# stevenabreu7/SparseRNNs

Hardware: AMD Instinct MI355X
Metric: frames/sec at w8a16 S5 dim_scale=0.5 (NDNS shape), bit-exact vs CPU fxprun (higher is better)
Workload: dtype int32

## Files before the change

### include/s5fxp.h

```cpp
#ifndef S5FXP_H
#define S5FXP_H

#include <stddef.h>
#include <stdint.h>

#ifdef __cplusplus
extern "C" {
#endif

#define S5FXP_VERSION 108

enum {
    S5FXP_OK = 0,
    S5FXP_EBADARG = -1,
    S5FXP_ENEGSHIFT = -2,
    S5FXP_EUNSUPPORTED = -3,
    S5FXP_EHIP = -4,
    S5FXP_EWORKSPACE = -5
};

enum { S5FXP_FLOOR = 0, S5FXP_CEIL = 1, S5FXP_ROUND = 2 };

int s5fxp_version(void);
const char *s5fxp_strerror(int code);
// ... 94 lines not shown
typedef struct {
    int32_t *pre_s5;
    int32_t *u;
    int32_t *Bu_re, *Bu_im;
    int32_t *xs_re, *xs_im;
    int32_t *ys;
    int32_t *out2;
    int32_t *out2_sigmoid;
    int32_t *post_GLU;
    int32_t *residadd;
} s5fxp_layer_trace;

size_t s5fxp_model_blob_bytes(const s5fxp_model_desc *desc);

enum { S5FXP_MODEL_DEFAULT = 0, S5FXP_MODEL_FORCE_DENSE = 1, S5FXP_MODEL_FORCE_CSR = 2, S5FXP_MODEL_FORCE_GENERIC = 4,
       S5FXP_MODEL_NO_RESID_FOLD = 8 };
int s5fxp_model_create(const s5fxp_model_desc *desc, void *dev_blob, size_t blob_bytes, int flags, void *stream,
                       s5fxp_model **out);
void s5fxp_model_destroy(s5fxp_model *m);

size_t s5fxp_workspace_bytes(const s5fxp_model *m, int B, int L);

#define S5FXP_STATUS_WORDS 128
enum { S5FXP_PATH_GENERIC = 1, S5FXP_PATH_FUSED = 2, S5FXP_PATH_STEP = 3 };
enum {
    S5FXP_ST_NEGSHIFT = 1,
    S5FXP_ST_NEGEXP = 2,
    S5FXP_ST_WIDE_STATE = 4,
    S5FXP_ST_WIDE_INPUT = 8,
    S5FXP_ST_REDO = 16
};
// ... 50 lines not shown
```

### sparsernns_amd/_lib.py

```python
from __future__ import annotations

import ctypes as C
import os

import torch

_HERE = os.path.dirname(os.path.abspath(__file__))
LIB_PATH = os.environ.get("S5FXP_LIB") or os.path.join(_HERE, "libs5fxp.so")

I32P = C.POINTER(C.c_int32)
VOIDP = C.c_void_p

S5FXP_OK, S5FXP_EBADARG, S5FXP_ENEGSHIFT, S5FXP_EUNSUPPORTED, S5FXP_EHIP, S5FXP_EWORKSPACE = 0, -1, -2, -3, -4, -5
ST_NEGSHIFT, ST_NEGEXP, ST_WIDE_STATE, ST_WIDE_INPUT, ST_REDO = 1, 2, 4, 8, 16
FWD_DEFER_REDO, FWD_EXACT, FWD_NO_PAIR = 1, 2, 4
STATUS_WORDS = 128
PATH_GENERIC, PATH_FUSED, PATH_STEP = 1, 2, 3
STEP_MAX_ROWS = 32
STREAM_MAX_HOPS = 32
MODEL_DEFAULT, MODEL_FORCE_DENSE, MODEL_FORCE_CSR, MODEL_FORCE_GENERIC, MODEL_NO_RESID_FOLD = 0, 1, 2, 4, 8


class DenseDesc(C.Structure):
    _fields_ = [("K", C.c_int32), ("M", C.c_int32), ("weight", I32P), ("bias", I32P)] + [
        (n, C.c_int32) for n in ("w_bits", "w_exp", "b_bits", "b_exp", "inp_bits", "inp_exp", "out_bits", "out_exp")]


class SSMDesc(C.Structure):
    _fields_ = [("H", C.c_int32), ("P", C.c_int32)] + [
        (n, I32P) for n in ("A_re", "A_im", "B_re", "B_im", "C_re", "C_im", "D")] + [
        (n, C.c_int32) for n in (
            "A_re_bits", "A_re_exp", "A_im_bits", "A_im_exp", "B_re_bits", "B_re_exp", "B_im_bits", "B_im_exp",
            "C_re_bits", "C_re_exp", "C_im_bits", "C_im_exp", "D_bits", "D_exp",
            "u_bits", "u_exp", "Bu_re_bits", "Bu_re_exp", "Bu_im_bits", "Bu_im_exp",
            "x_re_bits", "x_re_exp", "x_im_bits", "x_im_exp", "y_bits", "y_exp")]
# ... 116 lines not shown
```

### sparsernns_amd/csrc/mfma_bn.hpp

```cpp
#pragma once
#include "mfma_proj.hpp"

namespace s5 {

struct StatusInit {
    int32_t path;
    int32_t rk[15];
    int32_t slots[15];
    int32_t stream[15];
};
__global__ __launch_bounds__(256) void k_clear2(int32_t *a, int na, int32_t *b, int nb, StatusInit si, int n_layers, GroupOff go)
{
    gshift(a, (int64_t)blockIdx.y * go.status);
    gshift(b, (int64_t)blockIdx.y * go.ws);
    for (int i = blockIdx.x * 256 + threadIdx.x; i < na + nb; i += gridDim.x * 256) {
        if (i < na) {
            int32_t v = 0;
            if (i == 2) v = si.path;
            else if (i >= 8 && (i & 7) == 5 && (i - 8) / 8 < n_layers) v = si.rk[(i - 8) / 8];
            else if (i >= 8 && (i & 7) == 6 && (i - 8) / 8 < n_layers) v = si.slots[(i - 8) / 8];
            else if (i >= 8 && (i & 7) == 7 && (i - 8) / 8 < n_layers) v = si.stream[(i - 8) / 8];
            a[i] = v;
        } else b[i - na] = 0;
    }
// ... 470 lines not shown
__device__ __forceinline__ uint32_t pk_mul_sat(uint32_t a, uint32_t m)
{
    uint32_t r;
    asm("v_pk_mad_i16 %0, %1, %2, 0 clamp" : "=v"(r) : "v"(a), "v"(m));
    return r;
}
__device__ __forceinline__ uint32_t sum_u16_pair(const SumU16 &p, uint32_t z, uint32_t s)
{
    const uint32_t a = pk_mul_sat(pk_mul_sat(z, p.mz), p.mz2), b = pk_mul_sat(pk_mul_sat(s, p.ms), p.ms2);
    const uint32_t m = pk_max(a, pk_sub_sat(0u, b));
    uint32_t r;
    asm("v_pk_add_u16 %0, %1, %2" : "=v"(r) : "v"(m), "v"(b));
    return r;
}

enum { ROW_GENERIC = 0, ROW_PACKED = 1, ROW_SHIFTED = 2 };
struct Bn16Row {
    uint32_t m[4], iv[4];
    int32_t arm;
    uint32_t mulx, mulc, crp;
    int32_t shx1, l1, r1, rs2, cl, cr;
    int32_t xb, b1, b2, cbits;
};

__host__ __device__ __forceinline__ int bn16_row_arm(int xb, int mb, int ib, int b1, int b2, int cbits, int shx1, int l1, int r1, int cl, int cr)
{
    const bool w16 = (xb == 16 || (shx1 == 0 && xb < 16)) && mb <= 16 && ib <= 16 && b1 == 16 && b2 == 16 && cbits == 16 &&
                     shx1 <= 14 && l1 == 0 && cl <= 14 && cr <= 15;
    return !w16 ? ROW_GENERIC : r1 == 0 ? ROW_PACKED : ROW_SHIFTED;
}
// ... 61 lines not shown
    const int16_t *x;
    MfmaW w;
    int32_t *bq;
    int16_t *u;
    int32_t *tr_bu_re, *tr_bu_im, *tr_pre_s5, *tr_u;
    int64_t N;
    int32_t L, TB, H, P;
    int32_t rs_re, rs_im, bre_bits, bim_bits, sh_re, sh_im;
    int32_t t_lo, t_len;
    int32_t k_re;
    int32_t no_u;
    int32_t live_slots;
    const float *ext;
    int32_t ext_reps;
    int32_t *status, *status_exps;
};

}
```

### sparsernns_amd/csrc/mfma_fused.hpp

```cpp
#pragma once
#include "proj_p.hpp"

namespace s5 {

using v2i16 = __attribute__((ext_vector_type(2))) short;

struct CGateArgs {
    const int16_t *u;
    BnArgs bn;
    const int16_t *skip;
    const int32_t *xs;
    MfmaW w_re, w_im;
    MfmaW w_o2;
    const int32_t *D;
    const int32_t *bias_eff;
    int16_t *z;
    int32_t *tr_ys, *tr_out2, *tr_sig, *tr_z;
    int64_t N;
    int32_t L, TB, H;
    int32_t rs_re, rs_im, rs_d, y_bits, y_exp;
    int32_t xmax;
    int32_t conv, inp_bits, inp_exp, rs_o2, out_bits, out_exp;
    int32_t sig_x, sig_y;
    int32_t lut[8];
// ... 41 lines not shown
        w[0] = b0 ? r01 : w[0]; w[1] = b0 ? w[1] : r01;
        w[2] = b0 ? r23 : w[2]; w[3] = b0 ? w[3] : r23;
    }
    {
        const int32_t r02 = quad_xchg<0x4E>(b1 ? w[0] : w[2]), r13 = quad_xchg<0x4E>(b1 ? w[1] : w[3]);
        w[0] = b1 ? r02 : w[0]; w[2] = b1 ? w[2] : r02;
        w[1] = b1 ? r13 : w[1]; w[3] = b1 ? w[3] : r13;
    }
}


constexpr int SIGTAB_WORDS = 2 * 7 * 64;
constexpr int SIGDIR_MAX_BITS = 12, SIGDIR_BYTES = 2 << SIGDIR_MAX_BITS;
__host__ __device__ __forceinline__ int sigdir_lds_bytes(int bits) { return ((2 << bits) + 15) & ~15; }

template <int KS, int NT, bool TRACE, bool S16 = false, bool DIRECT = false, int FTP = 64, bool WIDE = false, bool PAIR = false, bool PK16 = false,
          bool GBN = false, bool UREC = false>
#ifndef S5_CGATE_HID
#define S5_CGATE_HID 0
#endif
#ifndef S5_CGATE_COAL
#define S5_CGATE_COAL 1
#endif
#ifndef S5_CGATE_LB
#define S5_CGATE_LB 4
#endif
__global__ __launch_bounds__(FTP * 2 * NT, NT == 3 && KS == 1 && !WIDE ? S5_CGATE_LB : 3) void k_cgate_p(const CGateArgs a_k, GroupOff go)
{
    constexpr bool FOLD = false;
#include "mfma_fused_body.inc"
}
struct CGateFoldArgs : CGateArgs {};
template <int KS, int NT, bool TRACE, bool S16, bool DIRECT, int FTP, bool WIDE, bool PAIR, bool PK16, bool GBN, bool UREC>
__global__ __launch_bounds__(FTP * 2 * NT, NT == 3 && KS == 1 && !WIDE ? S5_CGATE_LB : 3) void k_cgate_p(const CGateFoldArgs a_k, GroupOff go)
{
    constexpr bool FOLD = true;
#include "mfma_fused_body.inc"
}

}
```

### sparsernns_amd/csrc/mfma_fused_body.inc

```
    CGateArgs a = a_k;
    {
        const int64_t g = blockIdx.y;
        gshift(a.u, g * go.ws); gshift(a.skip, g * go.ws); gshift(a.xs, g * go.ws); gshift(a.z, g * go.ws);
        gshift(a.skip_e.dyn, g * go.ws); gshift(a.dynw, g * go.ws); gshift(a.run_if, g * go.ws); gshift(a.status, g * go.status);
        if constexpr (GBN || UREC) { gshift(a.bn.dyn, g * go.ws); gshift(a.bn.xe.dyn, g * go.ws); }
    }
    static_assert(!GBN || (PK16 && !TRACE && !WIDE), "the BatchNorm rides on the packed-epilogue kernel only");
    static_assert(!UREC || (S5_CGATE_COAL && PK16 && !TRACE && !WIDE && !GBN && !(S5_CGATE_HID && S16 && PAIR && KS * NT < 24)),
                  "u is rebuilt in the row tiles' staging: COAL only");
    constexpr int P = 32 * KS, H = shape_channels(NT), HP = 32 * NT, FT = FTP, NW = (FT / 32) * NT, NTHR = 64 * NW;
    constexpr bool RAGGED = H != HP;
    constexpr int KPS = 2 * P + 16, KPX = HP + 16;
    constexpr int NU = 1, SUBSTEP = 0;
    constexpr int ITEMS = (FT / 4) * P, ROUNDS = (ITEMS + NTHR - 1) / NTHR;
    constexpr bool HID = S5_CGATE_HID && S16 && PAIR && PK16 && !WIDE && !TRACE && KS * NT < 24;
    extern __shared__ __attribute__((aligned(16))) int8_t smem[];
    int32_t *csr = reinterpret_cast<int32_t *>(smem), *csi = csr + HP, *Dl = csi + HP, *cs2 = Dl + HP, *be = cs2 + HP, *lutp = be + HP;
    int32_t *sigt = lutp + 8;
    const int16_t *sigd = reinterpret_cast<const int16_t *>(sigt);
    constexpr int NPL = WIDE ? 4 : 2;
    int8_t *Sbase = reinterpret_cast<int8_t *>(sigt) + (DIRECT ? sigdir_lds_bytes(a.sigdir_bits) : 4 * SIGTAB_WORDS);
    int8_t *Sl = Sbase, *Sh = Sbase + (NPL - 1) * FT * KPS, *Xh = Sbase + NPL * FT * KPS, *Xl = Xh + FT * KPX;
    float *red = reinterpret_cast<float *>(Xl + FT * KPX);
    int32_t *bntab = reinterpret_cast<int32_t *>(red + 48);
// ... 35 lines not shown
    } else {
        for (int i = threadIdx.x; i < (14 << a.sig_x); i += NTHR) sigt[i] = a.sigtab[i];
    }
    Bn16 bn{};
    if constexpr (GBN) bn = bn16_setup(a.bn, *a.bn.dyn, bntab, H);
    std::conditional_t<UREC, Bn16Row, int> brow{};
    if constexpr (UREC) brow = bn16_row_setup(a.bn, *a.bn.dyn, 8 * (int)(threadIdx.x % VPF));
    const int dsh = a.out_exp - a.sig_x, dbias = 1 << (a.sigdir_bits - 1);
    const int skip_e = a.skip_e.get();
    const float kz = ldexpf(1.f, skip_e - a.res_exp);
    const v4i *usum_lds = reinterpret_cast<const v4i *>(red + 8);
    if constexpr (FOLD) {
        if (threadIdx.x == 0) {
            const SumU16 us = sum_u16_setup_exps(a.res_exp, skip_e);
            *reinterpret_cast<v4i *>(red + 8) = v4i{(int)us.mz, (int)us.mz2, (int)us.ms, (int)us.ms2};
        }
    }
    const int sx = a.sig_x, S = 1 << sx;
    const int cv_l = a.conv && a.inp_exp > a.y_exp ? a.inp_exp - a.y_exp : 0, cv_r = a.conv && a.y_exp > a.inp_exp ? a.y_exp - a.inp_exp : 0;
    const int cv_b1 = a.conv && a.inp_exp != a.y_exp ? a.y_bits : 32, cv_b2 = a.conv && a.y_bits > a.inp_bits ? a.inp_bits : 32;
    const int cv_b = cv_b1 < cv_b2 ? cv_b1 : cv_b2;
    const int lq_l = a.l_exp > a.y_exp ? a.l_exp - a.y_exp : 0, lq_r = a.y_exp > a.l_exp ? a.y_exp - a.l_exp : 0;
    uint32_t xrange = 0;
    v2i16 pmax = {0, 0}, pmin = {0, 0};
    float mx[3] = {0.f, 0.f, 0.f};
    const int ch0 = 32 * ct + 4 * h;
    v2i uq[NU][4], sq[NU][4];
    v4i urow[COAL && !UREC ? NVC : 1], srow[COAL ? NVC : 1];
    auto load_tile = [&](v4i(&dst)[COAL ? NVC : 1], const int16_t *src, const TileWalk<FT> &tw) {
        const int64_t b = tw.b;
        const int t = tw.t(sr), nv = tw.nvalid(sr);
        const char *base = reinterpret_cast<const char *>(src + (b * a.L + t) * H);
// ... 97 lines not shown
            }
        }
    };
    auto tiles_in_urec = [&](auto arm_c) {
        constexpr int ARM = decltype(arm_c)::value;
#pragma unroll
        for (int i = 0; i < NVC; ++i) {
            const int v = threadIdx.x + NTHR * i, f = v / VPF, og = v % VPF;
            if (!NVC_FULL && v >= FT * VPF) break;
            int8_t *cu = Ut + f * TROW + 16 * og, *cs_ = St + f * TROW + 16 * og;
            if (zb_prev) {
                v2i z0 = *reinterpret_cast<const v2i *>(cu), z1 = *reinterpret_cast<const v2i *>(cu + 8);
                if constexpr (FOLD) fold_z(z0, z1, cs_);
                if (f < nvalid_prev) *reinterpret_cast<v4i *>(zb_prev + 2u * (unsigned)(f * H + 8 * og)) = v4i{z0[0], z0[1], z1[0], z1[1]};
            }
            const v4i uv = bn16_row8<ARM>(brow, srow[i]);
            *reinterpret_cast<v2i *>(cu) = v2i{uv[0], uv[1]};
            *reinterpret_cast<v2i *>(cu + 8) = v2i{uv[2], uv[3]};
            *reinterpret_cast<v2i *>(cs_) = v2i{srow[i][0], srow[i][1]};
            *reinterpret_cast<v2i *>(cs_ + 8) = v2i{srow[i][2], srow[i][3]};
        }
    };

    prologue_loads_done();
    for (int64_t tile = blockIdx.x; tile < tiles; tile += gridDim.x, walk.advance()) {
        const int64_t b0 = walk.b;
        const int t0 = walk.t(sr), nvalid = walk.nvalid(sr);
        const TileWalk<FT> walk_next = walk.next();
        const int64_t n0 = b0 * a.L + t0;
        char *zb = reinterpret_cast<char *>(a.z + n0 * H);
// ... 312 lines not shown
```

### sparsernns_amd/csrc/proj_p.hpp

```cpp
#pragma once
#ifdef S5_PHASE_PROF
__device__ long long g_phase_prof[2048 * 8];
#define PHASE_DECL unsigned prof_last, prof_a0 = 0, prof_a1 = 0, prof_a2 = 0, prof_a3 = 0, prof_a4 = 0, prof_a5 = 0, prof_a6 = 0, prof_a7 = 0; \
    { unsigned long long t_; asm volatile("s_memtime %0\n\ts_waitcnt lgkmcnt(0)" : "=s"(t_)); prof_last = __builtin_amdgcn_readfirstlane((unsigned)t_); }
#define PHASE_MARK(i, reg) do { unsigned long long t_; asm volatile("v_cmp_eq_u32 vcc, %1, %1\n\ts_nop 0\n\ts_memtime %0\n\ts_waitcnt lgkmcnt(0)" : "=s"(t_) : "v"(reg) : "memory", "vcc"); \
    const unsigned tl_ = __builtin_amdgcn_readfirstlane((unsigned)t_); prof_a##i = __builtin_amdgcn_readfirstlane(prof_a##i + (tl_ - prof_last)); prof_last = tl_; } while (0)
#define PHASE_DUMP do { if (threadIdx.x == 0 && blockIdx.x < 2048) { long long *o_ = g_phase_prof + blockIdx.x * 8; o_[0] = prof_a0; o_[1] = prof_a1; o_[2] = prof_a2; o_[3] = prof_a3; \
    o_[4] = prof_a4; o_[5] = prof_a5; o_[6] = prof_a6; o_[7] = prof_a7; } } while (0)
#else
#define PHASE_DECL
#define PHASE_MARK(i, reg)
#define PHASE_DUMP
#endif
#define PHASE_DECL_F
#define PHASE_MARK_F(i, reg)
#define PHASE_DUMP_F
#include "mfma_bn.hpp"

namespace s5 {

__host__ __device__ constexpr int shape_channels(int NT) { return (NT == 2 || NT == 5) ? 32 * NT - 16 : 32 * NT; }

template <int HC, int HP, int KP>
__device__ __forceinline__ void zero_plane_tail(int8_t *base, int rows)
// ... 108 lines not shown
    if (wsub == 0 && h == 0) {
        const int col = 32 * wct + r;
        int n = 0;
        for (int k = 0; k < H; ++k) {
            const int8_t wv = a.w.wt[(size_t)col * a.w.Kp + k];
            if (wv != 0 && n < ELLW) ell[col * ELLW + n++] = (uint16_t)(k | ((unsigned)(uint8_t)wv << 8));
        }
        for (int j = n; j < ELLW; ++j) ell[col * ELLW + j] = 0;
        atomicMax(ellmax + wct, n);
    }
#endif
    const LayerDyn d = a.ext ? bn_finalize_mm_body(a.bn, a.ext, H, const_cast<LayerDyn *>(a.bn.dyn), a.status, a.status_exps, a.bn.xe.get(), a.ext_reps,
                                                   blockIdx.x == 0)
                             : *a.bn.dyn;
    const Bn16 bn = bn16_setup(a.bn, d, tab, H);
    __syncthreads();

    prologue_loads_done();
    for (int it = 0; tile < tiles; tile += gridDim.x, ++it, walk.advance()) {
        const int64_t b0 = walk.b;
        const int t0 = walk.t(sr), nvalid = walk.nvalid(sr);
        const int64_t n0 = b0 * a.L + t0;
        char *ub = reinterpret_cast<char *>(a.u + n0 * H);
        int8_t *xh = Xh + (it & 1) * PLANE, *xl = Xl + (it & 1) * PLANE;
#pragma unroll
        for (int i = 0; i < NV; ++i) {
            const int v = threadIdx.x + NTHR * i, f = v / VPF, og = v % VPF;
            const int64_t n = n0 + f;
            int32_t xin[8], t[8], u[8];
            unpack8_i16(raw[i], xin);
            bn16_x4(bn, reinterpret_cast<const int32_t(&)[4]>(xin[0]), 8 * og, reinterpret_cast<int32_t(&)[4]>(t[0]),
                    reinterpret_cast<int32_t(&)[4]>(u[0]));
            bn16_x4(bn, reinterpret_cast<const int32_t(&)[4]>(xin[4]), 8 * og + 4, reinterpret_cast<int32_t(&)[4]>(t[4]),
                    reinterpret_cast<int32_t(&)[4]>(u[4]));
            if (f < nvalid && (TRACE || !a.no_u)) {
                const v2i p0 = pack4_i16(u[0], u[1], u[2], u[3]), p1 = pack4_i16(u[4], u[5], u[6], u[7]);
                *reinterpret_cast<v4i *>(ub + 2u * (unsigned)(f * H + 8 * og)) = v4i{p0[0], p0[1], p1[0], p1[1]};
                if (TRACE) {
#pragma unroll
                    for (int e = 0; e < 8; ++e) {
                        if (a.tr_pre_s5) a.tr_pre_s5[n * H + 8 * og + e] = t[e];
                        if (a.tr_u) a.tr_u[n * H + 8 * og + e] = u[e];
                    }
                }
// ... 856 lines not shown
```

### sparsernns_amd/csrc/s5fxp_fast.hpp

```cpp
#pragma once

namespace s5 {
struct StepParams;
}

struct MfmaWDev {
    MfmaW w{};
    const int32_t *bias_eff = nullptr;
};

struct FastLayer {
    MfmaWDev bproj, cre, cim, out2;
    MfmaWDev bproj_pair;
    const int32_t *Dpad = nullptr;
    const int32_t *sigtab = nullptr;
    const int16_t *sigdir = nullptr;
    int sigdir_bits = 0;
    bool bias16 = false;
    bool compact_ok = false;
    int n_live = 0;
    int c_slots = 0;
    MfmaWDev c_bproj, c_bproj_pair, c_cre, c_cim;
    ScanBounds c_bounds;
    const int32_t *c_a_re = nullptr, *c_a_im = nullptr;
// ... 279 lines not shown

struct LayerPlan {
    bool compact;
    Rung rung;
    int P;
    int ks;
    int live_slots;
    int stream_slots;
    int32_t bound;
    int32_t xmax;
    bool direct;
    bool pk16;
    bool gate_bn;
    bool gate_urec;
    bool resid_fold;
    GateForm gate;
    const MfmaW *w_bproj, *w_cre, *w_cim;
    const int32_t *a_re, *a_im;
};

LayerPlan plan_layer(const s5fxp_model *m, int li, int fwd_flags, bool traced, bool carry, bool fold)
{
    const LayerDev &l = m->layers[li];
    const FastLayer &fl = m->fast->layers[li];
    const s5fxp_ssm_desc &s = l.sd;
    const FastShape sh = fast_shape(m->H, m->P);
    LayerPlan p{};
    p.compact = fl.compact_ok && !m->cfg.no_compact && !traced && !carry;
    p.rung = select_rung(m, li, fwd_flags, traced, p.compact);
    const Rung &r = p.rung;
// ... 37 lines not shown

template <int SM> auto bproj_kernel(const FastShape &sh, int ks)
{
    return nt_kernel(sh.nt, [&](auto n) {
        constexpr int NT = decltype(n)::value;
        return ks_kernel<NT>(ks, [](auto k) { return k_bproj_p<NT, bproj_waves_of<NT>(), false, SM, 2 * decltype(k)::value>; });
    });
}
inline auto bproj_traced_kernel(const FastShape &sh)
{
    return nt_kernel(sh.nt, [](auto n) { constexpr int NT = decltype(n)::value; return k_bproj_p<NT, bproj_waves_of<NT>(), true>; });
}

using GateKernel = void (*)(const CGateArgs, GroupOff);
using GateFoldKernel = void (*)(const CGateFoldArgs, GroupOff);
template <bool S16, bool DIR, bool PAIR, bool PK16> GateKernel cgate_kernel(const LayerPlan &p, const FastShape &sh)
{
    return nt_kernel(sh.nt, [&](auto n) -> GateKernel {
        constexpr int NT = decltype(n)::value;
        if constexpr (PK16 && NT == 3) {
            if (p.gate == GATE_FT32 && p.gate_urec)
                return ks_kernel<3>(p.ks, [](auto k) -> GateKernel { return k_cgate_p<decltype(k)::value, 3, false, S16, DIR, 32, false, PAIR, true, false, true>; });
            if (p.gate == GATE_FT32)
                return ks_kernel<3>(p.ks, [](auto k) -> GateKernel { return k_cgate_p<decltype(k)::value, 3, false, S16, DIR, 32, false, PAIR, true>; });
            if (p.gate == GATE_GBN)
                return ks_kernel<3>(p.ks, [](auto k) -> GateKernel { return k_cgate_p<decltype(k)::value, 3, false, S16, DIR, 64, false, PAIR, true, true>; });
        }
        return ks_kernel<NT>(p.ks, [](auto k) -> GateKernel { return k_cgate_p<decltype(k)::value, NT, false, S16, DIR, 64, false, PAIR, PK16>; });
    });
}
// ... 70 lines not shown
    const int dec_resid = bn_ext && fold && !traces && !cfg.no_dec_resid ? m->n_layers - 1 : -1;
    int64_t per_group(int64_t cap, int64_t floor_) const { return G > 1 ? std::max<int64_t>(cap / G, floor_) : cap; }
    const int64_t tiles64 = (N + 63) / 64, seq_tiles64 = (int64_t)B * ((L + 63) / 64);
    const unsigned grid_enc = grid_for(tiles64, per_group(cfg.cap_enc, 64)), grid_dec = grid_for(tiles64, per_group(cfg.cap_dec, 64));
    const int64_t cap_bproj = per_group(cfg.cap_bproj, 128);
    const unsigned grid_bproj = grid_for(seq_tiles64, sh.wide ? std::max<int64_t>(cap_bproj / 2, 1) : cap_bproj);
    const unsigned grid_gate = grid_for(seq_tiles64, per_group(cfg.cap_cgate, 64)), grid_gate_exact = grid_for(seq_tiles64, 512);
    const unsigned grid_gate32 = grid_for((int64_t)B * ((L + 31) / 32), std::max<int64_t>(cfg.cap_cgate32 / G, 1));
    const int64_t rm_step = 4 * (RESID_THREADS / (H / 8)), rm_iters = (N + rm_step - 1) / rm_step;
    const int64_t rm_per = std::min(std::max<int64_t>(1, ((int64_t(1) << 31) / (2 * H)) / rm_step),
                                    (rm_iters + per_group(cfg.cap_resid, 64) - 1) / per_group(cfg.cap_resid, 64));
    const int64_t rm_span = rm_per * rm_step;
    const unsigned rm_grid = (unsigned)((rm_iters + rm_per - 1) / rm_per);

    int16_t *h = I16(w.hA), *hn = I16(w.hB);
    int hb = m->enc.out_bits;
    DynExp he{m->enc.out_exp, nullptr};

    std::array<LayerPlan, 15> plan_layers() const
    {
        std::array<LayerPlan, 15> p{};
        for (int li = 0; li < m->n_layers; ++li) {
            p[li] = plan_layer(m, li, fwd_flags, traces != nullptr, state_in || state_out, fold);
            const int in_bits = li ? m->layers[li - 1].res_bits : m->enc.out_bits;
            p[li].resid_fold = p[li].gate_urec && defer && !traces && fold && m->layers[li].res_bits == 16 && in_bits == 16 &&
                               m->layers[li].res_exp >= 0 && m->layers[li].res_exp <= 16 && !(m->flags & S5FXP_MODEL_NO_RESID_FOLD);
        }
        return p;
    }
    int16_t *I16(size_t off) const { return reinterpret_cast<int16_t *>(ws + off); }
    int32_t *I32(size_t off) const { return reinterpret_cast<int32_t *>(ws + off); }
    const s5fxp_layer_trace *trace(int li) const { return traces ? &traces[li] : nullptr; }
    float *ext(int li) const { return reinterpret_cast<float *>(ws + w.ext) + (size_t)li * 2 * H * EXT_REPS; }
    int32_t *status_exps(int li) const { return status + 8 + 8 * li; }
    static hipEvent_t event(void **evs, int li, int k) { return evs ? (hipEvent_t)evs[2 * li + k] : nullptr; }

    template <class K, class... A>
    void launch(K kernel, unsigned grid, unsigned block, size_t smem, hipEvent_t ev0, hipEvent_t ev1, const A &...args) const
    {
        if (smem > 65536)
            (void)hipFuncSetAttribute(reinterpret_cast<const void *>(kernel), hipFuncAttributeMaxDynamicSharedMemorySize, (int)smem);
        if (ev0 && ev1) hipExtLaunchKernelGGL(kernel, dim3(grid, G), dim3(block), smem, st, ev0, ev1, 0, args..., go);
// ... 64 lines not shown
        const s5fxp_layer_trace *tr = trace(li);
        BprojM2Args a{};
        a.bn = bn; a.x = h; a.w = *p.w_bproj; a.bq = I32(w.bq); a.u = I16(w.u);
        a.tr_bu_re = tr ? tr->Bu_re : nullptr; a.tr_bu_im = tr ? tr->Bu_im : nullptr;
        a.tr_pre_s5 = tr ? tr->pre_s5 : nullptr; a.tr_u = tr ? tr->u : nullptr;
        a.N = N; a.L = L; a.TB = w.TB; a.H = H; a.P = p.P;
        a.rs_re = s.u_exp + s.B_re_exp - s.Bu_re_exp; a.rs_im = s.u_exp + s.B_im_exp - s.Bu_im_exp;
        a.bre_bits = s.Bu_re_bits; a.bim_bits = s.Bu_im_bits; a.sh_re = s.Bu_re_exp - s.x_re_exp; a.sh_im = s.Bu_im_exp - s.x_im_exp;
        a.k_re = 65536 - (1 << (16 - s.A_re_exp));
        a.live_slots = p.live_slots;
        a.no_u = (p.gate_bn || p.gate_urec) && defer ? 1 : 0;
        if (fold) {
            a.ext = ext(li);
            a.ext_reps = EXT_REPS; a.status = status; a.status_exps = status_exps(li);
        }
        a.t_lo = 0; a.t_len = L;
#ifdef S5_BPROJ_CSR
        const size_t smem = 16 * (size_t)sh.hp + 4 * 64 * (size_t)(sh.hp + 16) + 2 * (size_t)(2 * m->P) * S5_BPROJ_CSR + 64;
#else
        const size_t smem = 16 * (size_t)sh.hp + 4 * 64 * (size_t)(sh.hp + 16);
#endif
        const Rung &r = p.rung;
        auto kernel = tr ? bproj_traced_kernel(sh)
                         : r.pairl ? bproj_kernel<3>(sh, p.ks) : r.pair ? bproj_kernel<2>(sh, p.ks) : r.s16 ? bproj_kernel<1>(sh, p.ks) : bproj_kernel<0>(sh, p.ks);
        launch(kernel, grid_bproj, 64 * sh.bproj_waves, smem, nullptr, nullptr, a);
    }
    ScanQuadArgs quad_args(int li, const int32_t *run_if) const
    {
        const LayerPlan &p = layer[li];
        const s5fxp_ssm_desc &s = m->layers[li].sd;
// ... 45 lines not shown
        }
    }

    int gate(int li, const BnArgs &bn) const
    {
        const LayerPlan &p = layer[li];
        const Rung &r = p.rung;
        const LayerDev &l = m->layers[li];
        const FastLayer &fl = F.layers[li];
        const s5fxp_ssm_desc &s = l.sd;
        const DenseDev &o = l.out2;
        const s5fxp_layer_trace *tr = trace(li);
        LayerDyn *d = dyn + li;
        CGateArgs a{};
        a.u = I16(w.u); a.skip = h; a.xs = I32(w.xs); a.w_re = *p.w_cre; a.w_im = *p.w_cim; a.w_o2 = fl.out2.w;
        a.D = fl.Dpad; a.bias_eff = fl.out2.bias_eff; a.z = I16(w.z); a.sigtab = fl.sigtab; a.sigdir = fl.sigdir; a.sigdir_bits = fl.sigdir_bits; a.mx_slot = 8;
        a.tr_ys = tr ? tr->ys : nullptr; a.tr_out2 = tr ? tr->out2 : nullptr; a.tr_sig = tr ? tr->out2_sigmoid : nullptr;
        a.tr_z = tr ? tr->post_GLU : nullptr;
        a.N = N; a.L = L; a.TB = w.TB; a.H = H;
        a.rs_re = s.x_re_exp + s.C_re_exp - s.y_exp; a.rs_im = s.x_im_exp + s.C_im_exp - s.y_exp;
        a.rs_d = s.D_exp + s.u_exp - s.y_exp; a.y_bits = s.y_bits; a.y_exp = s.y_exp; a.xmax = p.xmax;
        a.conv = (s.y_bits > o.inp_bits || s.y_exp > o.inp_exp) ? 1 : 0; a.inp_bits = o.inp_bits; a.inp_exp = o.inp_exp;
        a.rs_o2 = (a.conv ? o.inp_exp : s.y_exp) + o.w_exp - o.out_exp;
        if (!shift_ok(a.rs_o2)) return S5FXP_ENEGSHIFT;
        a.out_bits = o.out_bits; a.out_exp = o.out_exp; a.sig_x = l.sig_x; a.sig_y = l.sig_y;
        std::memcpy(a.lut, l.lut, sizeof(a.lut));
        a.l_bits = l.l_bits; a.l_exp = l.l_exp; a.r_bits = l.r_bits; a.r_exp = l.r_exp; a.res_bits = l.res_bits;
        a.res_exp = l.res_exp; a.rs_gate = l.l_exp + l.r_exp - l.res_exp; a.skip_e = he; a.dynw = d; a.status = status;
        a.live_slots = p.live_slots;
        a.bad_bits = ST_WIDE_STATE | (defer ? ST_REDO : 0);
        a.bn = bn;
        a.t_lo = 0; a.t_len = L;
        const unsigned threads = sh.gate_threads;
        const size_t HP = sh.hp;
        void **evs = opts ? opts->gate_events : nullptr;
        const hipEvent_t gev0 = event(evs, li, 0), gev1 = event(evs, li, 1);
        const size_t sig_lds = p.direct ? (size_t)sigdir_lds_bytes(fl.sigdir_bits) : 4 * (size_t)SIGTAB_WORDS;
        if (exact) {
            for (int g = 0; g < G; ++g)
                if (int rc = hip_rc(hipMemsetAsync(reinterpret_cast<char *>(&d->redo) + (size_t)g * go.ws, 0xff, 4, st))) return rc;
        } else if (p.gate == GATE_FT32) {
            const size_t smem32 = 5 * HP * 4 + 32 + sig_lds + 2 * 32 * (size_t)(2 * p.P + 16) + 2 * 32 * (HP + 16) + 192 +
                                  2 * 32 * (2 * HP + 8);
            if (p.resid_fold) {
                CGateFoldArgs fa{};
                static_cast<CGateArgs &>(fa) = a;
                launch(gate_fold_kernel(p), grid_gate32, 192, smem32, gev0, gev1, fa);
            } else launch(gate_kernel(p, sh), grid_gate32, 192, smem32, gev0, gev1, a);
        } else {
            const size_t smem = 5 * HP * 4 + 32 + sig_lds + 2 * 64 * (size_t)(2 * p.P + 16) + 2 * 64 * (HP + 16) + 192 +
                                (p.gate_bn ? 16 * HP : 0) +
                                (p.pk16 && !p.gate_bn ? 2 * 64 * (2 * HP + 8) : 0);
            if (tr) launch(gate_traced_kernel(sh), grid_gate, threads, smem, nullptr, nullptr, a);
            else launch(gate_kernel(p, sh), grid_gate, threads, smem, gev0, gev1, a);
        }
        if (!defer) {
            if (r.quad) launch(k_scan_quad32_asm, (unsigned)((int64_t)B * p.P / 16), 64, 0, nullptr, nullptr, quad_args(li, &d->redo));
            CGateArgs e = a;
            e.run_if = &d->redo; e.mx_slot = 11; e.bad_bits = 0;
            const size_t smem_w = 5 * HP * 4 + 32 + 4 * (size_t)SIGTAB_WORDS + 4 * 64 * (size_t)(2 * p.P + 16) + 2 * 64 * (HP + 16) + 192;
            launch(gate_exact_kernel(p, sh, tr != nullptr), grid_gate_exact, threads, smem_w, nullptr, nullptr, e);
// ... 24 lines not shown
    ResidHead resid_head(int li) const
    {
        ResidHead hd{};
        hd.d = dyn + li; hd.res_exp = m->layers[li].res_exp; hd.skip_e = he; hd.redo_slot = redo_slot(); hd.status_exps = status_exps(li);
        hd.enable = fold ? 1 : 0;
        return hd;
    }

    void residual(int li)
    {
        const LayerDev &l = m->layers[li];
        const s5fxp_layer_trace *tr = trace(li);
        if (bn_ext) {
            const bool more = li + 1 < m->n_layers;
            const int ext_reps = (more && fold) ? EXT_REPS : 1;
            launch(layer[li].resid_fold ? k_resid_minmax16<true, true> : k_resid_minmax16<true, false>, rm_grid, RESID_THREADS, 0,
                   nullptr, nullptr, (const int16_t *)I16(w.z), (const int16_t *)h, hn,
                   tr ? tr->residadd : nullptr, N, H, rm_span, l.res_bits, hb, resid_head(li), more ? ext(li + 1) : nullptr, ext_reps,
                   status);
        } else {
            hipLaunchKernelGGL(k_resid16, dim3(ew_grid(NH / 4)), dim3(256), 0, st, (const int16_t *)I16(w.z),
                               (const int16_t *)h, hn, tr ? tr->residadd : nullptr, NH, l.res_bits, hb, (const LayerDyn *)(dyn + li));
        }
        std::swap(h, hn);
        hb = l.res_bits;
        he = DynExp{0, &dyn[li].res.eo};
    }

    void decoder(void *y) const
    {
        const DenseDev &e = m->dec;
        DecResid dz{};
        DecArgs a{};
        a.x = h; a.y = reinterpret_cast<int32_t *>(y); a.w = F.dec.w; a.bias_eff = F.dec.bias_eff; a.N = N; a.H = H; a.M = e.M;
        a.xb = hb; a.xe = he; a.inp_bits = e.inp_bits; a.inp_exp = e.inp_exp; a.w_exp = e.w_exp;
        a.out_bits = e.out_bits; a.out_exp = e.out_exp; a.status = status;
        if (dec_resid >= 0) {
            const LayerDev &l = m->layers[dec_resid];
            dz.z = I16(w.z); dz.res_bits = l.res_bits; dz.skip_bits = hb; dz.hd = resid_head(dec_resid);
            a.xb = l.res_bits;
            if (layer[dec_resid].resid_fold) {
                dz.usum = 1;
                a.x = I16(w.z);
            }
        }
        const size_t smem = 2 * 64 * (size_t)(sh.hp + 16);
        auto kernel = nt_kernel(sh.nt, [&](auto n) {
            constexpr int NT = decltype(n)::value;
            return f32 ? (dec_resid >= 0 ? k_dec_pf<NT, true> : k_dec_pf<NT, false>) : (dec_resid >= 0 ? k_dec_p<NT, true> : k_dec_p<NT, false>);
        });
        launch(kernel, grid_dec, 384, smem, nullptr, nullptr, a, dz);
    }
};

int forward_fast(const s5fxp_model *m, const void *x, int x_bits, int x_exp, int B, int L, void *y, void *workspace,
                 int32_t *status, const s5fxp_layer_trace *traces, const s5fxp_forward_opts *opts, hipStream_t st, int G = 1,
                 size_t ws_stride = 0, bool f32 = false)
{
    FusedForward f{m, opts, traces, status, st, G, B, L, reinterpret_cast<char *>(workspace), ws_stride, f32};
    int rc;
    f.clear_status();
    if ((rc = f.encoder(x, x_bits, x_exp))) return rc;
    if (!f.stage_ok("encoder", -1)) return S5FXP_EHIP;
    for (int li = 0; li < m->n_layers; ++li) {
        const BnArgs bn = make_bn(m->layers[li], f.hb, f.he, f.dyn + li);
        if ((rc = f.bn_exponents(li, bn))) return rc;
        f.bproj(li, bn);
        if (!f.stage_ok("B projection", li)) return S5FXP_EHIP;
        f.recurrence(li);
        if (!f.stage_ok("recurrence", li)) return S5FXP_EHIP;
        if ((rc = f.gate(li, bn))) return rc;
        if (!f.stage_ok("gate kernel", li)) return S5FXP_EHIP;
        if ((rc = f.res_exponent(li))) return rc;
        if (li == f.dec_resid) break;
        f.residual(li);
        if (!f.stage_ok("residual pass", li)) return S5FXP_EHIP;
    }
    f.decoder(y);
    if (!f.stage_ok("decoder", -1)) return S5FXP_EHIP;
    return launch_rc();
}
// ... 3 lines not shown
```

Measured before the change: 720.6 million.

## Defer residual resolve into next layer's B-projection and gate kernels

When two consecutive layers both use the folded residual, the residual pass becomes a read-only min/max kernel over the unresolved u16 sum. Its output buffer is not written; instead the pointer is swapped and the resolve (shift, clamp, saturating multiply) is applied lazily as the next layer's B-projection and gate kernels read the skip. This removes a full write of the hidden activation per layer. In exchange it adds packed-u16 resolve arithmetic to the consumers and restricts the path to particular kernel configurations, returning unsupported otherwise.

```diff
diff --git a/include/s5fxp.h b/include/s5fxp.h
--- a/include/s5fxp.h
+++ b/include/s5fxp.h
@@ -132,7 +132,7 @@
 size_t s5fxp_model_blob_bytes(const s5fxp_model_desc *desc);
 
 enum { S5FXP_MODEL_DEFAULT = 0, S5FXP_MODEL_FORCE_DENSE = 1, S5FXP_MODEL_FORCE_CSR = 2, S5FXP_MODEL_FORCE_GENERIC = 4,
-       S5FXP_MODEL_NO_RESID_FOLD = 8 };
+       S5FXP_MODEL_NO_RESID_FOLD = 8, S5FXP_MODEL_NO_RESID_LAZY = 16 };
 int s5fxp_model_create(const s5fxp_model_desc *desc, void *dev_blob, size_t blob_bytes, int flags, void *stream,
                        s5fxp_model **out);
 void s5fxp_model_destroy(s5fxp_model *m);
diff --git a/sparsernns_amd/_lib.py b/sparsernns_amd/_lib.py
--- a/sparsernns_amd/_lib.py
+++ b/sparsernns_amd/_lib.py
@@ -18,7 +18,7 @@
 PATH_GENERIC, PATH_FUSED, PATH_STEP = 1, 2, 3
 STEP_MAX_ROWS = 32
 STREAM_MAX_HOPS = 32
-MODEL_DEFAULT, MODEL_FORCE_DENSE, MODEL_FORCE_CSR, MODEL_FORCE_GENERIC, MODEL_NO_RESID_FOLD = 0, 1, 2, 4, 8
+MODEL_DEFAULT, MODEL_FORCE_DENSE, MODEL_FORCE_CSR, MODEL_FORCE_GENERIC, MODEL_NO_RESID_FOLD, MODEL_NO_RESID_LAZY = 0, 1, 2, 4, 8, 16
 
 
 class DenseDesc(C.Structure):
diff --git a/sparsernns_amd/csrc/mfma_bn.hpp b/sparsernns_amd/csrc/mfma_bn.hpp
--- a/sparsernns_amd/csrc/mfma_bn.hpp
+++ b/sparsernns_amd/csrc/mfma_bn.hpp
@@ -508,6 +508,147 @@
     return r;
 }
 
+enum { RES_GENERIC = 0, RES_RIGHT = 1 };
+struct ResolveU16 {
+    uint32_t shr, m1, m2;
+    int32_t arm;
+};
+__host__ __device__ __forceinline__ ResolveU16 resolve_u16_setup(int post)
+{
+    const int lsh = post > 0 ? post : 0, rsh = post < 0 ? -post : 0;
+    ResolveU16 p;
+    p.shr = 0x10001u * (uint32_t)(rsh & 15);
+    p.m1 = rsh > 15 ? 0u : 0x10001u << (lsh < 14 ? lsh : 14);
+    p.m2 = lsh > 14 ? 0x20002u : 0x10001u;
+    p.arm = lsh == 0 && rsh <= 15 ? RES_RIGHT : RES_GENERIC;
+    return p;
+}
+__device__ __forceinline__ uint32_t pk_lshr(uint32_t a, uint32_t s)
+{
+    uint32_t r;
+    asm("v_pk_lshrrev_b16 %0, %1, %2" : "=v"(r) : "v"(s), "v"(a));
+    return r;
+}
+__device__ __forceinline__ uint32_t pk_min_u(uint32_t a, uint32_t b)
+{
+    uint32_t r;
+    asm("v_pk_min_u16 %0, %1, %2" : "=v"(r) : "v"(a), "v"(b));
+    return r;
+}
+__device__ __forceinline__ uint32_t pk_max_u(uint32_t a, uint32_t b)
+{
+    uint32_t r;
+    asm("v_pk_max_u16 %0, %1, %2" : "=v"(r) : "v"(a), "v"(b));
+    return r;
+}
+template <int ARM = RES_GENERIC>
+__device__ __forceinline__ uint32_t resolve_u16_pair(const ResolveU16 &p, uint32_t u)
+{
+    const uint32_t t = pk_min_u(pk_lshr(u, p.shr), 0x7fff7fffu);
+    if constexpr (ARM == RES_RIGHT) return t;
+    else return pk_mul_sat(pk_mul_sat(t, p.m1), p.m2);
+}
+
+struct ResidLazyArgs {
+    const int16_t *u;
+    int64_t N, span;
+    int32_t H, res_bits;
+    ResidHead hd;
+    float *ext;
+    int32_t ext_reps;
+    int32_t *status;
+};
+template <bool RESID, bool USUM>
+__global__ __launch_bounds__(RESID_THREADS, 5) void k_resid_minmax16(ResidLazyArgs a, GroupOff go)
+{
+    static_assert(RESID && USUM, "the read-only pass exists for the one-plane residual add");
+    const int64_t gws = (int64_t)blockIdx.y * go.ws, gst = (int64_t)blockIdx.y * go.status;
+    const int16_t *__restrict__ u = reinterpret_cast<const int16_t *>(reinterpret_cast<const char *>(a.u) + gws);
+    ResidHead hd = a.hd;
+    float *ext = a.ext;
+    int32_t *status = a.status;
+    gshift(ext, gws); gshift_nn(hd.d, gws); gshift(hd.skip_e.dyn, gws); gshift_nn(hd.status_exps, gst); gshift_nn(status, gst);
+    __shared__ uint32_t smin[RESID_THREADS * 4], smax[RESID_THREADS * 4];
+    __shared__ AddCb sp;
+    const int H = a.H, G = H >> 3, R = RESID_THREADS / G;
+    const int g = threadIdx.x % G, rl = threadIdx.x / G;
+    const int64_t lo_n = (int64_t)blockIdx.x * a.span;
+    const int cnt = rl < R ? (int)((lo_n + a.span < a.N ? lo_n + a.span : a.N) - lo_n) : 0;
+    const char *ub = reinterpret_cast<const char *>(u + lo_n * H);
+    const unsigned rowb = 2u * (unsigned)H, toff = (unsigned)rl * rowb + 16u * (unsigned)g, kstep = (unsigned)R * rowb;
+    auto fetch = [&](v4i(&q)[4], int i0) {
+#pragma unroll
+        for (int k = 0; k < 4; ++k)
+            if (i0 + k * R + rl < cnt)
+                q[k] = __builtin_nontemporal_load(reinterpret_cast<const v4i *>(ub + toff + (unsigned)(i0 / R) * kstep + (unsigned)k * kstep));
+    };
+    v4i qa[4];
+    const int step = 4 * R;
+    if (rl < cnt) fetch(qa, 0);
+    AddCb p{};
+    if (hd.enable) {
+        if (threadIdx.x == 0) {
+            sp = finalize_add_cb(hd.d->mx + (hd.d->redo ? hd.redo_slot : 8), hd.res_exp, hd.skip_e.get(), a.res_bits, status);
+            if (blockIdx.x == 0) {
+                hd.d->res = sp;
+                hd.status_exps[4] = sp.eo;
+            }
+        }
+        __syncthreads();
+        p = sp;
+    } else {
+        p = hd.d->res;
+    }
+    uint32_t lo[4] = {0xffffffffu, 0xffffffffu, 0xffffffffu, 0xffffffffu}, hi[4] = {0u, 0u, 0u, 0u};
+    for (int i0 = 0; i0 + rl < cnt; i0 += step) {
+#pragma unroll
+        for (int k = 0; k < 4; ++k) {
+            if (i0 + k * R + rl < cnt) {
+#pragma unroll
+                for (int e = 0; e < 4; ++e) {
+                    lo[e] = pk_min_u(lo[e], (uint32_t)qa[k][e]);
+                    hi[e] = pk_max_u(hi[e], (uint32_t)qa[k][e]);
+                }
+            }
+        }
+        if (i0 + step + rl < cnt) fetch(qa, i0 + step);
+    }
+    if (!ext) return;
+#pragma unroll
+    for (int e = 0; e < 4; ++e) {
+        smin[threadIdx.x * 4 + e] = lo[e];
+        smax[threadIdx.x * 4 + e] = hi[e];
+    }
+    __syncthreads();
+    {
+        const int items = 2 * H, parts = RESID_THREADS / items > 1 ? 2 : 1, per = R / parts;
+        const int item = threadIdx.x % items, part = threadIdx.x / items;
+        const bool is_max = item >= H;
+        const int c = is_max ? item - H : item;
+        int32_t v = is_max ? 0 : 65535;
+        if (part < parts) {
+            const uint16_t *src = reinterpret_cast<const uint16_t *>(is_max ? smax : smin);
+            for (int r = part * per; r < (part + 1) * per; ++r) {
+                const int32_t t = src[r * G * 8 + c];
+                v = is_max ? max(v, t) : min(v, t);
+            }
+        }
+        __syncthreads();
+        if (parts == 2 && part == 1) smin[item] = (uint32_t)v;
+        __syncthreads();
+        if (part == 0) {
+            if (parts == 2) {
+                const int32_t t = (int32_t)smin[item];
+                v = is_max ? max(v, t) : min(v, t);
+            }
+            v = resolve_u16(v, p.post > 0 ? p.post : 0, p.post < 0 ? -p.post : 0, sat_bounds(a.res_bits));
+            const int rep = a.ext_reps > 1 ? (int)(blockIdx.x % a.ext_reps) : 0;
+            atomicMax(reinterpret_cast<uint32_t *>(ext) + rep * 2 * H + item,
+                      __float_as_uint(is_max ? EXT_BIAS + (float)v : EXT_BIAS - (float)v));
+        }
+    }
+}
+
 enum { ROW_GENERIC = 0, ROW_PACKED = 1, ROW_SHIFTED = 2 };
 struct Bn16Row {
     uint32_t m[4], iv[4];
@@ -599,6 +740,7 @@
     const float *ext;
     int32_t ext_reps;
     int32_t *status, *status_exps;
+    const LayerDyn *lazy;
 };
 
 }
diff --git a/sparsernns_amd/csrc/mfma_fused.hpp b/sparsernns_amd/csrc/mfma_fused.hpp
--- a/sparsernns_amd/csrc/mfma_fused.hpp
+++ b/sparsernns_amd/csrc/mfma_fused.hpp
@@ -79,6 +79,12 @@
 constexpr int SIGDIR_MAX_BITS = 12, SIGDIR_BYTES = 2 << SIGDIR_MAX_BITS;
 __host__ __device__ __forceinline__ int sigdir_lds_bytes(int bits) { return ((2 << bits) + 15) & ~15; }
 
+struct CGateFoldArgs : CGateArgs {
+    const LayerDyn *skip_dyn;
+};
+__device__ __forceinline__ const LayerDyn *skip_dyn_of(const CGateArgs &) { return nullptr; }
+__device__ __forceinline__ const LayerDyn *skip_dyn_of(const CGateFoldArgs &a) { return a.skip_dyn; }
+
 template <int KS, int NT, bool TRACE, bool S16 = false, bool DIRECT = false, int FTP = 64, bool WIDE = false, bool PAIR = false, bool PK16 = false,
           bool GBN = false, bool UREC = false>
 #ifndef S5_CGATE_HID
@@ -95,7 +101,6 @@
     constexpr bool FOLD = false;
 #include "mfma_fused_body.inc"
 }
-struct CGateFoldArgs : CGateArgs {};
 template <int KS, int NT, bool TRACE, bool S16, bool DIRECT, int FTP, bool WIDE, bool PAIR, bool PK16, bool GBN, bool UREC>
 __global__ __launch_bounds__(FTP * 2 * NT, NT == 3 && KS == 1 && !WIDE ? S5_CGATE_LB : 3) void k_cgate_p(const CGateFoldArgs a_k, GroupOff go)
 {
diff --git a/sparsernns_amd/csrc/mfma_fused_body.inc b/sparsernns_amd/csrc/mfma_fused_body.inc
--- a/sparsernns_amd/csrc/mfma_fused_body.inc
+++ b/sparsernns_amd/csrc/mfma_fused_body.inc
@@ -73,8 +73,20 @@
         if (threadIdx.x == 0) {
             const SumU16 us = sum_u16_setup_exps(a.res_exp, skip_e);
             *reinterpret_cast<v4i *>(red + 8) = v4i{(int)us.mz, (int)us.mz2, (int)us.ms, (int)us.ms2};
-        }
-    }
+            const LayerDyn *sd = skip_dyn_of(a_k);
+            gshift(sd, (int64_t)blockIdx.y * go.ws);
+            const ResolveU16 rz = resolve_u16_setup(sd ? sd->res.post : 0);
+            *reinterpret_cast<v4i *>(red + 12) = v4i{(int)rz.shr, (int)rz.m1, (int)rz.m2, sd ? 1 : 0};
+        }
+    }
+    auto resolve_skip = [&](v4i &sv) {
+        const v4i rw = *reinterpret_cast<const v4i *>(red + 12);
+        if (__builtin_amdgcn_readfirstlane(rw[3])) {
+            const ResolveU16 rz{(uint32_t)rw[0], (uint32_t)rw[1], (uint32_t)rw[2], RES_GENERIC};
+#pragma unroll
+            for (int q = 0; q < 4; ++q) sv[q] = (int)resolve_u16_pair<RES_GENERIC>(rz, (uint32_t)sv[q]);
+        }
+    };
     const int sx = a.sig_x, S = 1 << sx;
     const int cv_l = a.conv && a.inp_exp > a.y_exp ? a.inp_exp - a.y_exp : 0, cv_r = a.conv && a.y_exp > a.inp_exp ? a.y_exp - a.inp_exp : 0;
     const int cv_b1 = a.conv && a.inp_exp != a.y_exp ? a.y_bits : 32, cv_b2 = a.conv && a.y_bits > a.inp_bits ? a.inp_bits : 32;
@@ -202,6 +214,7 @@
                 if constexpr (FOLD) fold_z(z0, z1, cs_);
                 if (f < nvalid_prev) *reinterpret_cast<v4i *>(zb_prev + 2u * (unsigned)(f * H + 8 * og)) = v4i{z0[0], z0[1], z1[0], z1[1]};
             }
+            if constexpr (FOLD) resolve_skip(srow[i]);
             const v4i uv = bn16_row8<ARM>(brow, srow[i]);
             *reinterpret_cast<v2i *>(cu) = v2i{uv[0], uv[1]};
             *reinterpret_cast<v2i *>(cu + 8) = v2i{uv[2], uv[3]};
diff --git a/sparsernns_amd/csrc/proj_p.hpp b/sparsernns_amd/csrc/proj_p.hpp
--- a/sparsernns_amd/csrc/proj_p.hpp
+++ b/sparsernns_amd/csrc/proj_p.hpp
@@ -146,6 +146,16 @@
                                                    blockIdx.x == 0)
                              : *a.bn.dyn;
     const Bn16 bn = bn16_setup(a.bn, d, tab, H);
+    constexpr bool LAZY = KS == 3 && !TRACE;
+    ResolveU16 rz{};
+    int lazy_arm = 0;
+    if constexpr (LAZY) {
+        if (a.lazy) {
+            gshift_nn(a.lazy, (int64_t)blockIdx.y * go.ws);
+            rz = resolve_u16_setup(a.lazy->res.post);
+            lazy_arm = 1 + rz.arm;
+        }
+    }
     __syncthreads();
 
     prologue_loads_done();
@@ -160,6 +170,15 @@
             const int v = threadIdx.x + NTHR * i, f = v / VPF, og = v % VPF;
             const int64_t n = n0 + f;
             int32_t xin[8], t[8], u[8];
+            if constexpr (LAZY) {
+                if (lazy_arm == 1 + RES_RIGHT) {
+#pragma unroll
+                    for (int e = 0; e < 4; ++e) raw[i][e] = (int)resolve_u16_pair<RES_RIGHT>(rz, (uint32_t)raw[i][e]);
+                } else if (lazy_arm) {
+#pragma unroll
+                    for (int e = 0; e < 4; ++e) raw[i][e] = (int)resolve_u16_pair<RES_GENERIC>(rz, (uint32_t)raw[i][e]);
+                }
+            }
             unpack8_i16(raw[i], xin);
             bn16_x4(bn, reinterpret_cast<const int32_t(&)[4]>(xin[0]), 8 * og, reinterpret_cast<int32_t(&)[4]>(t[0]),
                     reinterpret_cast<int32_t(&)[4]>(u[0]));
diff --git a/sparsernns_amd/csrc/s5fxp_fast.hpp b/sparsernns_amd/csrc/s5fxp_fast.hpp
--- a/sparsernns_amd/csrc/s5fxp_fast.hpp
+++ b/sparsernns_amd/csrc/s5fxp_fast.hpp
@@ -317,6 +317,7 @@
     bool gate_bn;
     bool gate_urec;
     bool resid_fold;
+    bool resid_lazy;
     GateForm gate;
     const MfmaW *w_bproj, *w_cre, *w_cim;
     const int32_t *a_re, *a_im;
@@ -384,6 +385,9 @@
 
 using GateKernel = void (*)(const CGateArgs, GroupOff);
 using GateFoldKernel = void (*)(const CGateFoldArgs, GroupOff);
+using ResidKernel = void (*)(const int16_t *, const int16_t *, int16_t *, int32_t *, int64_t, int, int64_t, int, int, ResidHead, float *, int,
+                             int32_t *, GroupOff);
+using ResidLazyKernel = void (*)(ResidLazyArgs, GroupOff);
 template <bool S16, bool DIR, bool PAIR, bool PK16> GateKernel cgate_kernel(const LayerPlan &p, const FastShape &sh)
 {
     return nt_kernel(sh.nt, [&](auto n) -> GateKernel {
@@ -484,6 +488,8 @@
     const unsigned rm_grid = (unsigned)((rm_iters + rm_per - 1) / rm_per);
 
     int16_t *h = I16(w.hA), *hn = I16(w.hB);
+    int16_t *zp = I16(w.z);
+    const LayerDyn *h_lazy = nullptr;
     int hb = m->enc.out_bits;
     DynExp he{m->enc.out_exp, nullptr};
 
@@ -496,6 +502,8 @@
             p[li].resid_fold = p[li].gate_urec && defer && !traces && fold && m->layers[li].res_bits == 16 && in_bits == 16 &&
                                m->layers[li].res_exp >= 0 && m->layers[li].res_exp <= 16 && !(m->flags & S5FXP_MODEL_NO_RESID_FOLD);
         }
+        for (int li = 0; li + 1 < m->n_layers; ++li)
+            p[li].resid_lazy = p[li].resid_fold && p[li + 1].resid_fold && !(m->flags & S5FXP_MODEL_NO_RESID_LAZY);
         return p;
     }
     int16_t *I16(size_t off) const { return reinterpret_cast<int16_t *>(ws + off); }
@@ -590,6 +598,7 @@
             a.ext = ext(li);
             a.ext_reps = EXT_REPS; a.status = status; a.status_exps = status_exps(li);
         }
+        a.lazy = h_lazy;
         a.t_lo = 0; a.t_len = L;
 #ifdef S5_BPROJ_CSR
         const size_t smem = 16 * (size_t)sh.hp + 4 * 64 * (size_t)(sh.hp + 16) + 2 * (size_t)(2 * m->P) * S5_BPROJ_CSR + 64;
@@ -665,7 +674,7 @@
         LayerDyn *d = dyn + li;
         CGateArgs a{};
         a.u = I16(w.u); a.skip = h; a.xs = I32(w.xs); a.w_re = *p.w_cre; a.w_im = *p.w_cim; a.w_o2 = fl.out2.w;
-        a.D = fl.Dpad; a.bias_eff = fl.out2.bias_eff; a.z = I16(w.z); a.sigtab = fl.sigtab; a.sigdir = fl.sigdir; a.sigdir_bits = fl.sigdir_bits; a.mx_slot = 8;
+        a.D = fl.Dpad; a.bias_eff = fl.out2.bias_eff; a.z = zp; a.sigtab = fl.sigtab; a.sigdir = fl.sigdir; a.sigdir_bits = fl.sigdir_bits; a.mx_slot = 8;
         a.tr_ys = tr ? tr->ys : nullptr; a.tr_out2 = tr ? tr->out2 : nullptr; a.tr_sig = tr ? tr->out2_sigmoid : nullptr;
         a.tr_z = tr ? tr->post_GLU : nullptr;
         a.N = N; a.L = L; a.TB = w.TB; a.H = H;
@@ -696,6 +705,7 @@
             if (p.resid_fold) {
                 CGateFoldArgs fa{};
                 static_cast<CGateArgs &>(fa) = a;
+                fa.skip_dyn = h_lazy;
                 launch(gate_fold_kernel(p), grid_gate32, 192, smem32, gev0, gev1, fa);
             } else launch(gate_kernel(p, sh), grid_gate32, 192, smem32, gev0, gev1, a);
         } else {
@@ -750,15 +760,28 @@
         if (bn_ext) {
             const bool more = li + 1 < m->n_layers;
             const int ext_reps = (more && fold) ? EXT_REPS : 1;
-            launch(layer[li].resid_fold ? k_resid_minmax16<true, true> : k_resid_minmax16<true, false>, rm_grid, RESID_THREADS, 0,
-                   nullptr, nullptr, (const int16_t *)I16(w.z), (const int16_t *)h, hn,
+            if (layer[li].resid_lazy) {
+                ResidLazyArgs a{};
+                a.u = zp; a.N = N; a.span = rm_span; a.H = H; a.res_bits = l.res_bits; a.hd = resid_head(li);
+                a.ext = ext(li + 1); a.ext_reps = ext_reps; a.status = status;
+                launch(static_cast<ResidLazyKernel>(k_resid_minmax16<true, true>), rm_grid, RESID_THREADS, 0, nullptr, nullptr, a);
+                std::swap(h, zp);
+                h_lazy = dyn + li;
+                hb = l.res_bits;
+                he = DynExp{0, &dyn[li].res.eo};
+                return;
+            }
+            launch(layer[li].resid_fold ? static_cast<ResidKernel>(k_resid_minmax16<true, true>) : static_cast<ResidKernel>(k_resid_minmax16<true, false>),
+                   rm_grid, RESID_THREADS, 0,
+                   nullptr, nullptr, (const int16_t *)zp, (const int16_t *)h, hn,
                    tr ? tr->residadd : nullptr, N, H, rm_span, l.res_bits, hb, resid_head(li), more ? ext(li + 1) : nullptr, ext_reps,
                    status);
         } else {
-            hipLaunchKernelGGL(k_resid16, dim3(ew_grid(NH / 4)), dim3(256), 0, st, (const int16_t *)I16(w.z),
+            hipLaunchKernelGGL(k_resid16, dim3(ew_grid(NH / 4)), dim3(256), 0, st, (const int16_t *)zp,
                                (const int16_t *)h, hn, tr ? tr->residadd : nullptr, NH, l.res_bits, hb, (const LayerDyn *)(dyn + li));
         }
         std::swap(h, hn);
+        h_lazy = nullptr;
         hb = l.res_bits;
         he = DynExp{0, &dyn[li].res.eo};
     }
@@ -773,11 +796,11 @@
         a.out_bits = e.out_bits; a.out_exp = e.out_exp; a.status = status;
         if (dec_resid >= 0) {
             const LayerDev &l = m->layers[dec_resid];
-            dz.z = I16(w.z); dz.res_bits = l.res_bits; dz.skip_bits = hb; dz.hd = resid_head(dec_resid);
+            dz.z = zp; dz.res_bits = l.res_bits; dz.skip_bits = hb; dz.hd = resid_head(dec_resid);
             a.xb = l.res_bits;
             if (layer[dec_resid].resid_fold) {
                 dz.usum = 1;
-                a.x = I16(w.z);
+                a.x = zp;
             }
         }
         const size_t smem = 2 * 64 * (size_t)(sh.hp + 16);
@@ -801,6 +824,7 @@
     for (int li = 0; li < m->n_layers; ++li) {
         const BnArgs bn = make_bn(m->layers[li], f.hb, f.he, f.dyn + li);
         if ((rc = f.bn_exponents(li, bn))) return rc;
+        if (f.h_lazy && (f.sh.nt != 3 || traces || !f.layer[li].resid_fold)) return S5FXP_EUNSUPPORTED;
         f.bproj(li, bn);
         if (!f.stage_ok("B projection", li)) return S5FXP_EHIP;
         f.recurrence(li);
```

New measurement: 743.8 million (median of 6 runs). +3.2%, better.
